# iglu-contest/gridworld

Hardware: AMD Instinct MI355X
Metric: env-steps/sec (render=False, vector_state) at N parallel envs, 1/2/4/8 GPU (higher is better)
Workload: dtype f64

## Files before the change

gridworld_amd/csrc/render/igw_render_obs.hip:

```cpp
#include <stdio.h>

#include "igw_render_obs_stage.h"

namespace {

constexpr int kAgentBytes = 64;

constexpr int kSinkSlots = 2048;
__device__ uint4 g_sink[kSinkSlots * (kChunk * 3 / 16)];

__global__ __launch_bounds__(kThreads) void igw_obs_pov_kernel(const uint8_t* __restrict__ agent,
                                                           const int8_t* __restrict__ grid,
                                                           const uint32_t* __restrict__ occ, ObsOut ob,
                                                           const uint32_t* __restrict__ atlas, int side,
                                                           uint8_t* __restrict__ out, int W, int H) {
    const int tid = threadIdx.x;
    const int64_t env = blockIdx.x;
    if (tid < kGridStride / 16)
        s_grid4[tid] = reinterpret_cast<const uint4*>(grid + env * kGridStride)[tid];
    else if (tid >= 128 && tid < 128 + kOccWords / 4)
        s_occ4[tid - 128] = reinterpret_cast<const uint4*>(occ + env * kOccWords)[tid - 128];
    const double* pose = reinterpret_cast<const double*>(agent + env * kAgentBytes);
    const int wh = W * H, c0 = blockIdx.y * kChunk;
    uint8_t* dst = out;
    int64_t frame = env;
    if (!out) {
        const unsigned slot = (blockIdx.x * gridDim.y + blockIdx.y) % (unsigned)kSinkSlots;
        dst = reinterpret_cast<uint8_t*>(reinterpret_cast<uintptr_t>(g_sink) + (uintptr_t)slot * (kChunk * 3) -
                                         (uintptr_t)c0 * 3);
        frame = 0;
    }
    render_frame<false>(pose, lds_occ(), lds_grid(), s_stage4, atlas, side, dst, frame, W, H, 3);
    ob.store(reinterpret_cast<const uint8_t*>(s_stage4), env, wh, c0, min(kChunk, wh - c0));
}

thread_local char g_err[512] = "";

int fail(int code, const char* what, const char* detail = "") {
    snprintf(g_err, sizeof(g_err), "igw_render_pov_obs: %s%s", what, detail);
    return code;
}

bool aligned(const void* p, uintptr_t a) { return (reinterpret_cast<uintptr_t>(p) & (a - 1)) == 0; }

bool have_device() {
    static int seen = 0;
    if (!seen) {
        int cnt = 0;
        if (hipGetDeviceCount(&cnt) != hipSuccess || cnt < 1) return false;
        seen = 1;
    }
    return true;
}

}

#ifndef IGW_RENDER_OBS_BUILD_ID
#define IGW_RENDER_OBS_BUILD_ID "igw-render-obs-build-id:unstamped"
#endif

static_assert(sizeof(igw_render_obs) == IGW_RENDER_OBS_BYTES, "include/igw_render_obs.h: IGW_RENDER_OBS_BYTES");

extern "C" {

const char* igw_render_obs_build_id(void) { return &IGW_RENDER_OBS_BUILD_ID[sizeof("igw-render-obs-build-id:") - 1]; }
const char* igw_render_obs_last_error(void) { return g_err; }

int igw_render_pov_obs(const void* agent, const int8_t* grid, const uint32_t* occ, int32_t n, const uint8_t* atlas,
                       int32_t atlas_side, uint8_t* out, int32_t width, int32_t height, const igw_render_obs* obs,
                       void* stream) {
    if (!obs) return fail(IGW_RENDER_ERR_INVALID, "obs is NULL");
    if (n < 0) return fail(IGW_RENDER_ERR_INVALID, "n must be >= 0");
    if (n > 0 && (!agent || !grid || !occ || !atlas)) return fail(IGW_RENDER_ERR_INVALID, "null buffer");
    if (!aligned(agent, 8) || !aligned(grid, 16) || !aligned(occ, 16) || !aligned(atlas, 4))
        return fail(IGW_RENDER_ERR_INVALID, "agent must be 8-byte, grid and occ 16-byte, atlas 4-byte aligned");
    if (obs->dtype < IGW_OBS_U8 || obs->dtype > IGW_OBS_F32)
        return fail(IGW_RENDER_ERR_INVALID, "obs.dtype must be an IGW_OBS_*");
    if (obs->stack < 1 || obs->stack > IGW_RENDER_MAX_STACK)
        return fail(IGW_RENDER_ERR_INVALID, "obs.stack must be in 1..8");
    if (!isfinite(obs->scale) || !isfinite(obs->bias))
        return fail(IGW_RENDER_ERR_INVALID, "obs.scale and obs.bias must be finite");
    if (obs->dtype == IGW_OBS_U8 && (obs->scale != 1.f || obs->bias != 0.f))
        return fail(IGW_RENDER_ERR_INVALID, "IGW_OBS_U8 takes scale 1 and bias 0");
    if (n > 0 && !obs->data) return fail(IGW_RENDER_ERR_INVALID, "obs.data is NULL");
    if (!aligned(obs->data, obs->dtype == IGW_OBS_U8 ? 1 : obs->dtype == IGW_OBS_F32 ? 4 : 2))
        return fail(IGW_RENDER_ERR_INVALID, "obs.data must be aligned to its element size");
    if (obs->restart && obs->restart_stride < 1)
        return fail(IGW_RENDER_ERR_INVALID, "obs.restart_stride must be >= 1");
    if (width < 1 || width > IGW_RENDER_MAX_SIDE || height < 1 || height > IGW_RENDER_MAX_SIDE)
        return fail(IGW_RENDER_ERR_INVALID, "width and height must be in 1..1024");
    if (atlas_side < 8 || atlas_side > IGW_RENDER_MAX_ATLAS || atlas_side % 8)
        return fail(IGW_RENDER_ERR_INVALID, "atlas_side must be a multiple of 8 in 8..256");
    if (!have_device())
        return fail(IGW_RENDER_ERR_NO_DEVICE, "no HIP device available (the renderer has no CPU fallback)");
    if (n == 0) return IGW_RENDER_OK;
    const ObsOut ob{obs->data, obs->restart, obs->restart_stride, obs->scale, obs->bias,
                    obs->dtype, obs->gray != 0, obs->stack, obs->fill != 0};
    const int chunks = (width * height + kChunk - 1) / kChunk;
    hipLaunchKernelGGL(igw_obs_pov_kernel, dim3((unsigned)n, (unsigned)chunks), dim3(kThreads), 0, (hipStream_t)stream,
                       static_cast<const uint8_t*>(agent), grid, occ, ob, reinterpret_cast<const uint32_t*>(atlas),
                       (int)atlas_side, out, (int)width, (int)height);
    const hipError_t e = hipGetLastError();
    if (e != hipSuccess) return fail(IGW_RENDER_ERR_HIP, "launch failed: ", hipGetErrorString(e));
    return IGW_RENDER_OK;
}

}
```

Baseline: 6.481 billion.

## Specialize POV obs renderer with occupied-bounds grid and slab-entry DDA

Replaces the generic render_frame call in the observation kernel with a dedicated obs_frame routine. Before any rays are cast, it computes a per-env bitmask of occupied x/y/z columns in shared memory using atomics. Each ray first clips to the grid's bounding slab, skips traversal entirely when the world is empty, and stops the DDA once it leaves the occupied range. This is meant to cut per-pixel traversal steps, at the cost of an extra barrier and an atomic reduction. It also stores a scratch word in the grid padding, which depends on that padding existing.

```diff
diff --git a/gridworld_amd/csrc/render/igw_render_obs.hip b/gridworld_amd/csrc/render/igw_render_obs.hip
--- a/gridworld_amd/csrc/render/igw_render_obs.hip
+++ b/gridworld_amd/csrc/render/igw_render_obs.hip
@@ -8,6 +8,177 @@
 
 constexpr int kSinkSlots = 2048;
 __device__ uint4 g_sink[kSinkSlots * (kChunk * 3 / 16)];
+
+constexpr int kAxesWord = (kCells + 3) / 4;
+static_assert(kAxesWord * 4 >= kCells && kAxesWord * 4 + 4 <= kGridStride, "the axes word lies in the grid's padding");
+
+__device__ __forceinline__ uint32_t occupied_axes(const uint32_t* s_occ, uint32_t* s_axes) {
+    const int tid = threadIdx.x;
+    if (tid < 99) {
+        const int yv = tid / 11, xv = tid - yv * 11;
+        const int bit = yv * 169 + (xv + 1) * 13 + 1, w = bit >> 5, sh = bit & 31;
+        uint32_t bits = s_occ[w] >> sh;
+        if (sh > 21) bits |= s_occ[w + 1] << (32 - sh);
+        bits &= 0x7ffu;
+        if (bits) atomicOr(s_axes, 1u << xv | 1u << (11 + yv) | bits << 20);
+    }
+    __syncthreads();
+    return __builtin_amdgcn_readfirstlane(*s_axes);
+}
+
+__device__ __forceinline__ void obs_frame(const double* pose, const uint32_t* s_occ, const int8_t* s_grid,
+                                          uint4* s_stage4, const uint32_t* atlas, int side, uint8_t* out,
+                                          int64_t frame, int W, int H) {
+    constexpr int C = 3;
+    const int tid = threadIdx.x;
+    const double ex = pose[0], ey = pose[1], ez = pose[2];
+    double sy, cy, sp, cp;
+    sincos(pose[3] * (M_PI / 180.0), &sy, &cy);
+    sincos(pose[4] * (M_PI / 180.0), &sp, &cp);
+    const float fx = (float)(sy * cp), fy = (float)sp, fz = (float)(-cy * cp);
+    const float rx = (float)cy, rz = (float)sy;
+    const float ux = (float)(-sy * sp), uy = (float)cp, uz = (float)(cy * sp);
+    const bool visible = fabs(ex) < 1e4 && fabs(ey) < 1e4 && fabs(ez) < 1e4 && isfinite(fx + fy + fz + ux + uy + uz);
+    const double oxd = visible ? floor(ex) : 0., oyd = visible ? floor(ey) : 0., ozd = visible ? floor(ez) : 0.;
+    const int ox = (int)oxd, oy = (int)oyd, oz = (int)ozd;
+    const float px0 = visible ? (float)(ex - oxd) : 0.f, py0 = visible ? (float)(ey - oyd) : 0.f,
+                pz0 = visible ? (float)(ez - ozd) : 0.f;
+    const float lox = -5.5f - (float)ox, loy = -1.5f - (float)oy, loz = -5.5f - (float)oz;
+    const float ground = -1.5f - (float)oy;
+    __syncthreads();
+    const uint32_t axes = occupied_axes(s_occ, reinterpret_cast<uint32_t*>(s_grid4) + kAxesWord);
+    const bool blocks = axes != 0u;
+    const uint32_t ax = axes & 0x7ffu, ay = (axes >> 11) & 0x1ffu, az = axes >> 20;
+    const int x0 = __ffs(ax) - 1, x1 = 31 - __clz(ax), y0 = __ffs(ay) - 1, y1 = 31 - __clz(ay), z0 = __ffs(az) - 1,
+              z1 = 31 - __clz(az);
+    uint8_t* stage = reinterpret_cast<uint8_t*>(s_stage4);
+
+    const int wh = W * H;
+    const int c0 = blockIdx.y * kChunk;
+    const int len = min(kChunk, wh - c0);
+    const int sub = side >> 3;
+    const float inv_h = 1.f / (float)H;
+    const int di = kThreads / W, dj = kThreads - di * W;
+    int i = (c0 + tid) / W, j = (c0 + tid) - i * W;
+    for (int q = tid; q < len; q += kThreads, i += di, j += dj) {
+        if (j >= W) { j -= W; i++; }
+        uint32_t rgba = IGW_RENDER_CLEAR_RGBA;
+        if (visible) {
+            const float a = (float)(2 * j + 1 - W) * inv_h, b = (float)(H - 2 * i - 1) * inv_h;
+            const float dx = fx + a * rx + b * ux, dy = fy + b * uy, dz = fz + a * rz + b * uz;
+            const float ix = 1.f / dx, iy = 1.f / dy, iz = 1.f / dz;
+            int face = -1, hx = 0, hy = 0, hz = 0;
+            float th = 0.f;
+            if (blocks) {
+                float t0 = 0.f, t1 = kFar;
+                int axis = -1;
+                bool miss = false;
+#define IGW_SLAB(P, D, I, LO, N, K)                                                       \
+                if (D != 0.f) {                                                           \
+                    float ta = (LO - P) * I, tb = (LO + N - P) * I;                       \
+                    if (ta > tb) { float s = ta; ta = tb; tb = s; }                       \
+                    if (ta > t0) { t0 = ta; axis = K; }                                   \
+                    t1 = fminf(t1, tb);                                                   \
+                } else if (P < LO || P > LO + N) miss = true;
+                IGW_SLAB(px0, dx, ix, lox, 11.f, 0)
+                IGW_SLAB(py0, dy, iy, loy, 9.f, 1)
+                IGW_SLAB(pz0, dz, iz, loz, 11.f, 2)
+#undef IGW_SLAB
+                if (!miss && t0 <= t1) {
+                    int cx = min(max((int)floorf(px0 + t0 * dx - lox), 0), 10);
+                    int cyy = min(max((int)floorf(py0 + t0 * dy - loy), 0), 8);
+                    int cz = min(max((int)floorf(pz0 + t0 * dz - loz), 0), 10);
+                    if (axis == 0) cx = dx > 0.f ? 0 : 10;
+                    if (axis == 1) cyy = dy > 0.f ? 0 : 8;
+                    if (axis == 2) cz = dz > 0.f ? 0 : 10;
+                    const int face_x = dx > 0.f ? kLeft : kRight, face_y = dy > 0.f ? kBottom : kTop,
+                              face_z = dz > 0.f ? kBack : kFront;
+                    int bit = cyy * 169 + (cx + 1) * 13 + (cz + 1);
+                    if (axis >= 0 && t0 >= kNear && ((s_occ[bit >> 5] >> (bit & 31)) & 1u)) {
+                        face = axis == 0 ? face_x : axis == 1 ? face_y : face_z;
+                        th = t0;
+                    }
+                    const int sx = dx > 0.f ? 1 : -1, syy = dy > 0.f ? 1 : -1, sz = dz > 0.f ? 1 : -1;
+                    const int endx = dx > 0.f ? x1 + 1 : x0 - 1, endy = dy > 0.f ? y1 + 1 : y0 - 1,
+                              endz = dz > 0.f ? z1 + 1 : z0 - 1;
+                    const bool past = (dx > 0.f ? cx >= endx : cx <= endx) || (dy > 0.f ? cyy >= endy : cyy <= endy) ||
+                                      (dz > 0.f ? cz >= endz : cz <= endz);
+                    float nx = dx != 0.f ? (lox + (float)(cx + (dx > 0.f)) - px0) * ix : INFINITY;
+                    float ny = dy != 0.f ? (loy + (float)(cyy + (dy > 0.f)) - py0) * iy : INFINITY;
+                    float nz = dz != 0.f ? (loz + (float)(cz + (dz > 0.f)) - pz0) * iz : INFINITY;
+                    for (int it = 0; !past && face < 0 && it < 30; ++it) {
+                        float t;
+                        int f;
+                        if (nx <= ny && nx <= nz) {
+                            t = nx; cx += sx; bit += 13 * sx; f = face_x;
+                            if (cx == endx) break;
+                            nx = (lox + (float)(cx + (dx > 0.f)) - px0) * ix;
+                        } else if (ny <= nz) {
+                            t = ny; cyy += syy; bit += 169 * syy; f = face_y;
+                            if (cyy == endy) break;
+                            ny = (loy + (float)(cyy + (dy > 0.f)) - py0) * iy;
+                        } else {
+                            t = nz; cz += sz; bit += sz; f = face_z;
+                            if (cz == endz) break;
+                            nz = (loz + (float)(cz + (dz > 0.f)) - pz0) * iz;
+                        }
+                        if (t > kFar) break;
+                        if (t >= kNear && ((s_occ[bit >> 5] >> (bit & 31)) & 1u)) { face = f; th = t; }
+                    }
+                    hx = cx; hy = cyy; hz = cz;
+                }
+            }
+            int col = -1, rowb = 0;
+            if (face >= 0) {
+                const float lx = px0 + th * dx - (lox + (float)hx), ly = py0 + th * dy - (loy + (float)hy),
+                            lz = pz0 + th * dz - (loz + (float)hz);
+                float u, v;
+                int cu, cv;
+                switch (face) {
+                    case kTop: u = lz; v = lx; cu = 0; cv = 1; break;
+                    case kBottom: u = lx; v = lz; cu = 1; cv = 0; break;
+                    case kLeft: u = lz; v = ly; cu = 0; cv = 0; break;
+                    case kRight: u = 1.f - lz; v = ly; cu = 0; cv = 0; break;
+                    case kFront: u = lx; v = ly; cu = 1; cv = 1; break;
+                    default: u = 1.f - lx; v = ly; cu = 1; cv = 1; break;
+                }
+                const int cell = hy * 121 + hx * 11 + hz;
+                int id = s_grid[cell];
+                id = id < 1 ? 1 : id > 6 ? 6 : id;
+                const int tile = id + 1;
+                col = (tile & 3) * 2 * sub + cu * sub + texel_index(u, sub);
+                rowb = (tile >> 2) * 2 * sub + cv * sub + texel_index(v, sub);
+            } else if (dy < 0.f && py0 > ground) {
+                const float t = (ground - py0) * iy;
+                if (t >= kNear && t <= kFar) {
+                    const float gx = px0 + t * dx + 0.5f, gz = pz0 + t * dz + 0.5f;
+                    const float fgx = floorf(gx), fgz = floorf(gz);
+                    const int qx = ox + (int)fgx, qz = oz + (int)fgz;
+                    if (qx >= -18 && qx <= 18 && qz >= -18 && qz <= 18) {
+                        const int tile = (qx >= -5 && qx <= 5 && qz >= -5 && qz <= 5) ? 0 : 1;
+                        col = tile * 2 * sub + texel_index(gz - fgz, 2 * sub);
+                        rowb = texel_index(gx - fgx, 2 * sub);
+                    }
+                }
+            }
+            if (col >= 0) rgba = atlas[(side - 1 - rowb) * side + col];
+        }
+        stage[3 * q] = (uint8_t)rgba;
+        stage[3 * q + 1] = (uint8_t)(rgba >> 8);
+        stage[3 * q + 2] = (uint8_t)(rgba >> 16);
+    }
+    __syncthreads();
+    const int nbytes = len * C;
+    uint8_t* dst = out + (frame * (int64_t)wh + c0) * C;
+    if (((reinterpret_cast<uintptr_t>(dst) | (uintptr_t)nbytes) & 15) == 0) {
+        for (int k = tid; k < nbytes / 16; k += kThreads) reinterpret_cast<uint4*>(dst)[k] = s_stage4[k];
+    } else if (((reinterpret_cast<uintptr_t>(dst) | (uintptr_t)nbytes) & 3) == 0) {
+        for (int k = tid; k < nbytes / 4; k += kThreads)
+            reinterpret_cast<uint32_t*>(dst)[k] = reinterpret_cast<const uint32_t*>(stage)[k];
+    } else {
+        for (int k = tid; k < nbytes; k += kThreads) dst[k] = stage[k];
+    }
+}
 
 __global__ __launch_bounds__(kThreads) void igw_obs_pov_kernel(const uint8_t* __restrict__ agent,
                                                            const int8_t* __restrict__ grid,
@@ -16,9 +187,11 @@
                                                            uint8_t* __restrict__ out, int W, int H) {
     const int tid = threadIdx.x;
     const int64_t env = blockIdx.x;
-    if (tid < kGridStride / 16)
-        s_grid4[tid] = reinterpret_cast<const uint4*>(grid + env * kGridStride)[tid];
-    else if (tid >= 128 && tid < 128 + kOccWords / 4)
+    if (tid < kGridStride / 16) {
+        uint4 cells = reinterpret_cast<const uint4*>(grid + env * kGridStride)[tid];
+        if (tid == kAxesWord / 4) (&cells.x)[kAxesWord % 4] = 0u;
+        s_grid4[tid] = cells;
+    } else if (tid >= 128 && tid < 128 + kOccWords / 4)
         s_occ4[tid - 128] = reinterpret_cast<const uint4*>(occ + env * kOccWords)[tid - 128];
     const double* pose = reinterpret_cast<const double*>(agent + env * kAgentBytes);
     const int wh = W * H, c0 = blockIdx.y * kChunk;
@@ -30,7 +203,7 @@
                                          (uintptr_t)c0 * 3);
         frame = 0;
     }
-    render_frame<false>(pose, lds_occ(), lds_grid(), s_stage4, atlas, side, dst, frame, W, H, 3);
+    obs_frame(pose, lds_occ(), lds_grid(), s_stage4, atlas, side, dst, frame, W, H);
     ob.store(reinterpret_cast<const uint8_t*>(s_stage4), env, wh, c0, min(kChunk, wh - c0));
 }
 
```

After: 6.464 billion. No clear change (-0.3%).
